# satoken/ractip

Measured on NVIDIA B200. Metric: shuffled pairs/sec, probability stage of --zscore=12 (McCaskill in/out x2 + unpaired windows x2 + two-strand McCaskill), higher is better.
Workload: dtype f64

## Files before the change

### ractip_b200/csrc/api.cu

```cuda
#include <cuda_runtime.h>

#include <algorithm>
#include <cstdio>
#include <cstdlib>
#include <string>
#include <utility>
#include <vector>

#include "dev_model.h"
#include "kernels.h"
#include "plan.h"
#include "ractip_prob.h"

using rp::Problem;

struct rp_ctx {
  int device = 0;
  int sm_count = 0;
  int ctas_per_sm = 0;
  int ctas_per_sm1 = 0;
  int up_ctas_per_sm = 0;
  size_t smem_optin = 0;
  rp::RouteSettings route;
  rp::DevModel* d_model = nullptr;
// ... 397 lines not shown
  CU(cudaEventRecord(ctx->ev[0], st));
  int launches = 0;
  if (p.n_band[0] && p.n_band[1]) CU(cudaEventRecord(ctx->ev_fork, st));
  for (int k = 0; k < 2; k++) {
    if (!p.n_band[k]) continue;
    rp::BatchDev db = d;
    db.order = b->d_order + (k ? p.n_band[0] : 0); db.nprob = p.n_band[k];
    db.counter = b->d_counter + 1 + k;
    db.ws = ctx->ws + p.ws_band[k]; db.slot_stride = p.band_slot[k]; db.nslots = p.band_grid[k];
    cudaStream_t ls = st;
    if (k == 1 && p.n_band[0]) {
      CU(cudaStreamWaitEvent(ctx->side_stream, ctx->ev_fork, 0));
      ls = ctx->side_stream;
    }
    if (p.dom_kind == k) CU(cudaEventRecord(ctx->ev_dom[0], ls));
    CU(rp::launch_band(db, p.band_grid[k], rp::BAND_THREADS[k], p.band_smem[k], ls));
    if (p.dom_kind == k) { CU(cudaEventRecord(ctx->ev_dom[1], ls)); ctx->dom_timed = true; }
    if (k == 0 && p.split_fetch) CU(cudaEventRecord(ctx->ev_main, st));
    if (ls != st) {
      CU(cudaEventRecord(ctx->ev_join, ls));
      CU(cudaStreamWaitEvent(st, ctx->ev_join, 0));
    }
    launches++;
  }
  if (p.up_mode == 1) {
    rp::BatchDev du = d;
    du.order = b->d_order + n_bandall + p.n_general; du.nprob = p.n_defer;
    du.counter = b->d_counter + 3;
    CU(rp::launch_unstru(du, p.up_grid, st));
    launches++;
  }
  if (p.n_mcc > 0) {
    if (p.dom_kind == 2) CU(cudaEventRecord(ctx->ev_dom[0], st));
    bool launched = false;
    for (int G = p.cluster; G && !launched; G = G == 16 ? 8 : 0) {
      const int ncl = std::max(1, std::min({p.n_mcc, p.grid, ctx->sm_count / G}));
      if (rp::launch_mcc_cluster(d, ncl, G, st) == cudaSuccess) launched = true;
      else cudaGetLastError();
    }
    if (!launched) CU(rp::launch_mcc(d, p.grid, p.mcc_minb, st));
    if (p.dom_kind == 2) { CU(cudaEventRecord(ctx->ev_dom[1], st)); ctx->dom_timed = true; }
    launches++;
  }
  if (p.n_duplex > 0) {
    CU(rp::launch_duplex(d, p.grid, st));
    launches++;
  }
  CU(cudaEventRecord(ctx->ev[1], st));
#ifdef RP_TUNE
  if (ctx->profile) {
    long long h[64];
    CU(cudaMemcpyAsync(h, ctx->d_prof, sizeof h, cudaMemcpyDeviceToHost, st));
    CU(cudaStreamSynchronize(st));
    static const char* names[32] = {"stage", "prologue", "prologue2", "inside_A", "inside_B", "generic_in", "generic_out", "outside_A", "outside_B", "write_bp", "un_hairpin", "un_gaps0", "un_gaps1", "un_domrows", "un_domcols", "un_mltab", "un_windows", "write_hp", "logz", "band_A", "band_B", "collect", "un_hairpin.cells(t0)", "un_hairpin.specials(t0)", "finish_in.loads(t0)", "finish_in.rest(t0)", "bandA_in.head(t0)", "bandA_in.main(t0)", "bandA_in.tail(t0)", "bandA_out.PR(t0)", "bandA_out.need(t0)", "bandA_out.ML(t0)"};
    long long tot = 0;
    for (int k = 0; k < 22; k++) tot += h[k];
    for (int k = 0; k < 32; k++)
      if (h[32 + k]) std::fprintf(stderr, "[rp_profile] %-11s %6.2f%%  calls %9lld  cycles/call %9.0f\n", names[k], 100.0 * h[k] / tot, h[32 + k], (double)h[k] / h[32 + k]);
  }
#endif
  ctx->timing.kernel_launches = launches;
  ctx->timing_pending = true;
  ctx->timed_copies = false;
  return RP_OK;
}

int rp_batch_sync(rp_batch* b) {
  if (!b) return RP_ERR_ARG;
  rp_ctx* ctx = b->ctx;
  CU(cudaStreamSynchronize(ctx->stream));
  return RP_OK;
}

int rp_batch_fetch_dense(rp_batch* b, float* out, size_t out_floats) {
  if (!b || !out) return RP_ERR_ARG;
  rp_ctx* ctx = b->ctx;
  const rp::BatchPlan& p = b->plan;
  if (out_floats < p.total_floats) return fail(ctx, RP_ERR_CAPACITY, "rp_batch_fetch_dense: buffer too small");
  CU(cudaSetDevice(ctx->device));
  CU(cudaEventRecord(ctx->ev[2], ctx->stream));
  if (p.total_floats && p.split_fetch) {
    const size_t pitch = p.pair_stride * sizeof(float);
    CU(cudaStreamWaitEvent(ctx->copy_stream, ctx->ev_main, 0));
    for (const auto& sc : p.sect_long)
      CU(cudaMemcpy2DAsync(out + sc.first, pitch, b->d_dense + sc.first, pitch, sc.second * sizeof(float), (size_t)b->n_pairs,
                           cudaMemcpyDeviceToHost, ctx->copy_stream));
    CU(cudaEventRecord(ctx->ev_copy, ctx->copy_stream));
    for (const auto& sc : p.sect_short)
      CU(cudaMemcpy2DAsync(out + sc.first, pitch, b->d_dense + sc.first, pitch, sc.second * sizeof(float), (size_t)b->n_pairs,
                           cudaMemcpyDeviceToHost, ctx->stream));
    CU(cudaStreamWaitEvent(ctx->stream, ctx->ev_copy, 0));
  } else if (p.total_floats) {
    CU(cudaMemcpyAsync(out, b->d_dense, p.total_floats * sizeof(float), cudaMemcpyDeviceToHost, ctx->stream));
  }
  CU(cudaEventRecord(ctx->ev[3], ctx->stream));
  CU(cudaStreamSynchronize(ctx->stream));
  ctx->timed_copies = true;
  return RP_OK;
}

}

namespace {
int sparse_prepare(rp_batch* b) {
  rp_ctx* ctx = b->ctx;
  const int np = b->n_pairs;
  if (b->d_spairs || np == 0) return RP_OK;
  std::vector<rp::SparsePair> sp(np);
  for (int p = 0; p < np; p++) {
// ... 175 lines not shown
```

### ractip_b200/csrc/mcc_core.h

```cpp
#ifndef RP_MCC_CORE_H
#define RP_MCC_CORE_H

#include <math.h>
#include <stdint.h>

#include "dev_model.h"

#ifdef __CUDACC__
#define RP_HD __host__ __device__ __forceinline__
#else
#define RP_HD inline
#endif

#ifdef RP_TUNE
#define RP_DBG(c) ((c).dbg)
#define RP_PROF(c) ((c).prof)
#else
#define RP_DBG(c) 0
#define RP_PROF(c) (static_cast<long long*>(nullptr))
#endif

namespace rp {

enum { KIND_LINEAR = 0, KIND_COFOLD = 1, KIND_DUPLEX = 2 };

struct Problem {
  int seq_off;
  int n;
  int cp;
  int kind;
  int pair;
  int which;
  int max_w;
  int n1, n2;
  long long out_bp;
  long long out_up;
  long long out_hp;
  float th_hy;
  int defer_up;
  long long ws_off;
};
constexpr int RP_JOB_UNPAIRED = 0x40000000;

enum {
  T_Q = 0, T_QQ, T_QM, T_QM1, T_QM2, T_QB, T_QBI, T_QB1N, T_QBAU,
  T_OUT, T_OUTI, T_OUT1N, T_OUTAU, T_MC, T_PR, T_PRML, T_PMLB, T_PL,
  T_DG, T_RR, T_LL, T_XX,
  T_QS, T_PRB, T_MLB,
  T_QMR, T_PRMLR,
  T_LIST,
  T_COUNT
};
enum {
  V_SCALE = 0, V_MLB, V_HPW, V_SP3, V_SP4, V_SP6, V_U0, V_U1,
  V_COUNT
};

constexpr int RP_MAX_N = 12000;
RP_HD size_t table_elems(int n) { return (size_t)n * (size_t)(n + 1) + 8; }
RP_HD size_t vector_elems(int n) { return (size_t)n + 8; }
RP_HD size_t slot_doubles(int n) { return T_COUNT * table_elems(n) + V_COUNT * vector_elems(n); }

struct Ctx {
  const DevModel* M;
  const uint8_t* S;
  int n, cp, ld, kind, max_w;
  double* ws;
  unsigned te, ve;
  double invZ;
  int dbg;
  long long* prof;
  RP_HD static constexpr unsigned ring_mask(int t) {
    return (t == T_PR || t == T_PL || t == T_PMLB) ? 1u : (t == T_QS || t == T_PRB || t == T_MLB) ? 15u : 0xffffffffu;
  }
  RP_HD unsigned off(int t, int d, int i) const { return (unsigned)t * te + ((unsigned)d & ring_mask(t)) * (unsigned)ld + (unsigned)i; }
  RP_HD double& tb(int t, int d, int i) const { return ws[off(t, d, i)]; }
  RP_HD double* ptr(int t, int d, int i) const { return ws + off(t, d, i); }
  RP_HD double* rptr(int t, int i, int j) const { return ws + ((unsigned)t * te + (unsigned)(i - 1) * (unsigned)ld + (unsigned)j); }
  RP_HD double& v(int vv, int k) const { return ws[(unsigned)T_COUNT * te + (unsigned)vv * ve + (unsigned)k]; }
  RP_HD int dstep() const { return ld; }
  RP_HD int pstep() const { return 1; }
  RP_HD int sraw(int i) const { return S[i]; }
};

RP_HD void bind_ctx(Ctx& c, const DevModel* M, const uint8_t* S, const Problem& p, double* ws) {
  c.M = M; c.S = S; c.n = p.n; c.cp = p.cp; c.ld = p.n + 1; c.kind = p.kind; c.max_w = p.max_w;
  c.ws = ws; c.te = (unsigned)table_elems(p.n); c.ve = (unsigned)vector_elems(p.n);
  c.invZ = 0;
  c.dbg = 0;
  c.prof = nullptr;
}
#define TB(c, t, d, i) ((c).tb(t, d, i))
#ifdef __CUDA_ARCH__
#define RP_ST_STREAM(ref, v) __stcs(&(ref), (v))
#else
#define RP_ST_STREAM(ref, v) ((ref) = (v))
#endif
#define VEC(c, vec_id, k) ((c).v(vec_id, k))

RP_HD uint16_t* listp(const Ctx& c) { return reinterpret_cast<uint16_t*>(c.ptr(T_LIST, 0, 0)); }
RP_HD uint16_t* posp(const Ctx& c) { return reinterpret_cast<uint16_t*>(c.ptr(T_LIST, 0, 0)) + c.te * 2; }

constexpr int BAND = TURN + 2;
constexpr int WIDE_MAX = 15;

constexpr int RP_SMEM_SEQ = 4096;
struct Shared {
  int T;
  double* part;
  double* grow;
  double* ghead_b;
  double* ghead_1;
  double* red;
  uint8_t* S;
  double* gtile;
  double* gpart;
};
constexpr int GS_ROW0 = 6, GS_NROWS = MAXLOOP - GS_ROW0 + 1;
RP_HD int gs_lt(int T) { return (T + MAXLOOP + 8 + 7) / 8 * 8; }
constexpr int GS_KINDS = 5;
RP_HD size_t gs_doubles(int T) { return (size_t)GS_KINDS * T + (size_t)GS_NROWS * gs_lt(T) + 8 * (size_t)T; }
RP_HD size_t part_doubles(int T, int W) {
  const size_t far = 2 * (size_t)W * T;
  return (W > BAND && gs_doubles(T) > far) ? gs_doubles(T) : far;
}
RP_HD size_t shared_bytes(int T, int W = BAND) {
  return sizeof(double) * (part_doubles(T, W) + (MAXLOOP + 1) * GROW_LD + 2 * GROW_LD + 128) + RP_SMEM_SEQ + 16;
}
RP_HD void carve_shared(Shared& sh, void* base, int T, int W = BAND) {
  sh.T = T;
  double* p = static_cast<double*>(base);
  sh.part = p; p += part_doubles(T, W);
// ... 1130 lines not shown
  }
}
template <int SIGN>
RP_HD void generic_items(const Ctx& c, const Shared& sh, int d, int i0, int C, int tid) {
  const int T = sh.T, LT = gs_lt(T), L8 = LT / 8;
  const GSplit gs = make_gsplit(C, T);
  const int warp = tid >> 5, lane = tid & 31;
  const int blk = warp / gs.wpb, bin = warp - blk * gs.wpb;
  if (blk >= gs.nb) return;
  const int g = blk * 32 + lane;
  const int smax = gs_smax(c.n, d, SIGN), nrows = smax - GS_ROW0 + 1;
  double tot[8];
#pragma unroll
  for (int r = 0; r < 8; r++) tot[r] = 0.;
  if (g < gs.NG) {
    for (int idx = bin; idx < nrows; idx += gs.wpb) {
      const int s = (idx & 1) ? GS_ROW0 + (idx >> 1) : smax - (idx >> 1);
      const double* row = sh.gtile + (size_t)(s - GS_ROW0) * LT + g;
#define RP_GX(cc) (((cc) & 7) * L8 + ((cc) >> 3))
      double win[8];
#pragma unroll
      for (int r = 0; r < 7; r++) win[r] = row[RP_GX(2 + r)];
      win[7] = 0.;
      const int nst = s - 3;
      int x = 0;
#pragma unroll 1
      for (; x + 8 <= nst; x += 8) {
#pragma unroll
        for (int u = 0; u < 8; u++) {
          win[(u + 7) & 7] = row[RP_GX(9 + u) + (x >> 3)];
          const double gv = sh.grow[(2 + x + u) * GROW_LD + (s - 2 - x - u)];
#pragma unroll
          for (int r = 0; r < 8; r++) tot[r] += gv * win[(u + r) & 7];
        }
      }
#pragma unroll
      for (int u = 0; u < 7; u++) {
        if (x + u < nst) {
          win[(u + 7) & 7] = row[RP_GX(9 + u) + (x >> 3)];
          const double gv = sh.grow[(2 + x + u) * GROW_LD + (s - 2 - x - u)];
#pragma unroll
          for (int r = 0; r < 8; r++) tot[r] += gv * win[(u + r) & 7];
        }
      }
#undef RP_GX
    }
  }
#pragma unroll
  for (int r = 0; r < 8; r++)
    if (8 * g + r < gs.cap) sh.gpart[(size_t)bin * gs.cap + 8 * g + r] = tot[r];
}

template <class C>
RP_HD void unstru_hairpin(C& c, int tid, int T) {
  const int n = c.n;
  const unsigned total = (unsigned)n * (unsigned)c.ld, ld = (unsigned)c.ld;
  for (unsigned x = tid; x < total; x += T) {
    const int d = (int)(x / ld), i = (int)(x - (unsigned)d * ld);
    if (i < 1 || i + d > n) continue;
    double v = 0.;
    if (d > TURN) {
      const double o = TB(c, T_OUT, d, i);
      if (o != 0.) v = o * hairpin(c, i, i + d, pair_type(base(c, i), base(c, i + d)));
    }
    TB(c, T_DG, d, i) = v;
  }
}
RP_HD int loop_class(int u1, int u2) {
  const int ul = u1 > u2 ? u1 : u2, us = u1 > u2 ? u2 : u1;
  if (us == 0) return ul >= 2 ? CLS_BULGE : CLS_SPECIAL;
  if (us == 1) return ul >= 3 ? CLS_1N : CLS_SPECIAL;
  return (us == 2 && (ul == 2 || ul == 3)) ? CLS_SPECIAL : CLS_GENERIC;
}

RP_HD int gap_special_slices(int n) { return n >= 48 ? 4 : 1; }
template <class C, class MT>
RP_HD void unstru_gap_specials(C& c, const MT& M, int tid, int T) {
  const int n = c.n;
  if (n < 7) return;
  const int nsl = gap_special_slices(n);
  const int items = (RP_DBG(c) & 4) ? 0 : 2 * 3 * nsl * n;
  for (int x = tid; x < items; x += T) {
    const int a = x % n + 1;
    int y = x / n;
    const int sl = y % nsl; y /= nsl;
    const int ug = y % 3 + 1, side = y / 3;
    const int b = a + ug + 1;
    double acc = 0.;
    if (b <= n) {
      if (side == 0) {
        const int p = a, k = b, u1 = ug, lmin = k + TURN + 1;
        const int sp1 = base(c, k - 1), si1 = base(c, p + 1);
        for (int u2 = 0; u2 <= 3; u2++) {
          if (loop_class(u1, u2) != CLS_SPECIAL) continue;
          const int lmax = n - 1 - u2, sidx = special_index(u1, u2);
          for (int l0 = lmin + sl; l0 <= lmax; l0 += 4 * nsl) {
            double qb[4], ou[4];
#pragma unroll
            for (int u = 0; u < 4; u++) {
              const int l = l0 + u * nsl;
              const bool on = l <= lmax;
              qb[u] = on ? TB(c, T_QB, l - k, k) : 0.;
              ou[u] = on ? TB(c, T_OUT, l + 1 + u2 - p, p) : 0.;
            }
            double w[4];
#pragma unroll
            for (int u = 0; u < 4; u++) {
              const int l = l0 + u * nsl <= lmax ? l0 + u * nsl : lmax, o = l + 1 + u2;
              w[u] = special_loop(M, sidx, pair_type(base(c, p), base(c, o)), rtype(pair_type(base(c, k), base(c, l))),
                                  si1, base(c, o - 1), sp1, base(c, l + 1));
            }
#pragma unroll
            for (int u = 0; u < 4; u++) acc += ou[u] * qb[u] * w[u];
          }
        }
      } else {
        const int l = a, o = b, u2 = ug;
        const int sq1 = base(c, l + 1), sj1 = base(c, o - 1);
        for (int u1 = 0; u1 <= 3; u1++) {
          if (loop_class(u1, u2) != CLS_SPECIAL) continue;
          const int pmax = l - TURN - 2 - u1, sidx = special_index(u1, u2);
          for (int p0 = 1 + sl; p0 <= pmax; p0 += 4 * nsl) {
            double qb[4], ou[4];
#pragma unroll
            for (int u = 0; u < 4; u++) {
              const int p = p0 + u * nsl;
              const bool on = p <= pmax;
              ou[u] = on ? TB(c, T_OUT, o - p, p) : 0.;
              qb[u] = on ? TB(c, T_QB, l - (p + 1 + u1), p + 1 + u1) : 0.;
            }
            double w[4];
#pragma unroll
            for (int u = 0; u < 4; u++) {
              const int p = p0 + u * nsl <= pmax ? p0 + u * nsl : pmax, k = p + 1 + u1;
              w[u] = special_loop(M, sidx, pair_type(base(c, p), base(c, o)), rtype(pair_type(base(c, k), base(c, l))),
                                  base(c, p + 1), sj1, base(c, k - 1), sq1);
            }
#pragma unroll
            for (int u = 0; u < 4; u++) acc += ou[u] * qb[u] * w[u];
          }
        }
      }
    }
    TB(c, T_RR, ((side * 3 + ug - 1) * nsl + sl), a) = acc;
  }
}

template <class C>
RP_HD void unstru_gaps(C& c, const double* gfull, int side, int tid, int T) {
  const int n = c.n, ds = c.dstep(), ps = c.pstep();
  const int items = (RP_DBG(c) & 4) ? 0 : n * (MAXLOOP + 1);
  const int tabO[3] = {T_OUTI, T_OUT1N, T_OUTAU};
  const int tabQ[3] = {T_QBI, T_QB1N, T_QBAU};
  for (int x = tid; x < items; x += T) {
    const int ug = x / n;
    const int a = x % n + 1;
    const int b = a + ug + 1;
    if (b > n || ug < 1) continue;
    double acc = 0.;
    if (side == 0) {
      const int p = a, k = b, u1 = ug;
      const int lmin = k + TURN + 1;
      for (int u2 = 0; u1 + u2 <= MAXLOOP;) {
        if (n - 1 - u2 < lmin) break;
        const int cls = loop_class(u1, u2);
        if (cls != CLS_SPECIAL) {
          int nu = 1;
          while (nu < 8 && u1 + u2 + nu <= MAXLOOP && loop_class(u1, u2 + nu) == cls && n - 1 - (u2 + nu) >= lmin) nu++;
          double av[8] = {0., 0., 0., 0., 0., 0., 0., 0.};
          const double* Q = c.ptr(tabQ[cls], lmin - k, k);
          const double* O = c.ptr(tabO[cls], lmin + 1 + u2 - p, p);
          const int cmain = n - 1 - (u2 + nu - 1) - lmin + 1;
          const int X = cmain + nu - 1;
          if (nu == 1) av[0] = dot_range(Q, ds, O, ds, 0, X, 0, 1);
          else multi_dot_slide(Q, ds, O, ds, X, 0, X - 1, av);
          for (int t = 0; t < nu; t++) acc += gfull[u1 * GROW_LD + u2 + t] * av[t];
          u2 += nu;
        } else {
          u2++;
        }
      }
    } else {
      const int l = a, o = b, u2 = ug;
      for (int u1 = 0; u1 + u2 <= MAXLOOP;) {
        if (l - TURN - 2 - u1 < 1) break;
        const int cls = loop_class(u1, u2);
        if (cls != CLS_SPECIAL) {
          int nu = 1;
          while (nu < 8 && u1 + nu + u2 <= MAXLOOP && loop_class(u1 + nu, u2) == cls && l - TURN - 2 - (u1 + nu) >= 1) nu++;
          double av[8] = {0., 0., 0., 0., 0., 0., 0., 0.};
          const double* O = c.ptr(tabO[cls], o - 1, 1);
          const double* Q = c.ptr(tabQ[cls], l - 2 - u1, 2 + u1);
          const int cmain = l - TURN - 2 - (u1 + nu - 1);
          if (cmain > 0) {
            const long st = ps - ds;
            const int X = cmain + nu - 1;
            if (nu == 1) {
              av[0] = dot_range(O + (long)(X - 1) * st, (int)-st, Q + (long)(X - 1) * st, (int)-st, 0, X, 0, 1);
            } else {
              double rv[8] = {0., 0., 0., 0., 0., 0., 0., 0.};
              multi_dot_slide(O + (long)(X - 1) * st, -st, Q + (long)(X + 6) * st, -st, X, 7, X + 6, rv);
#pragma unroll
              for (int t = 0; t < 8; t++) av[t] = rv[7 - t];
            }
          }
          for (int t = 0; t < nu; t++) acc += gfull[(u1 + t) * GROW_LD + u2] * av[t];
          u1 += nu;
        } else {
          u1++;
        }
      }
    }
    if (ug <= 3 && n >= 7) {
      const int nsl = gap_special_slices(n);
      for (int sl = 0; sl < nsl; sl++) acc += TB(c, T_RR, ((side * 3 + ug - 1) * nsl + sl), a);
    }
    TB(c, T_DG, b - a, a) += acc;
  }
}
template <class C>
RP_HD void unstru_dom_rows(C& c, int tid, int T) {
  const int n = c.n;
  for (int a = 1 + tid; a <= n; a += T) {
    double s = 0.;
    for (int b = n; b > a; b--) {
      s += TB(c, T_DG, b - a, a);
      TB(c, T_DG, b - a, a) = s;
    }
  }
}
template <class C>
RP_HD void unstru_dom_cols(C& c, int tid, int T) {
  const int n = c.n;
  for (int b = 2 + tid; b <= n; b += T) {
    double s = 0.;
    for (int a = 1; a < b; a++) {
      s += TB(c, T_DG, b - a, a);
      TB(c, T_DG, b - a, a) = s;
    }
  }
}
template <class C>
RP_HD void unstru_ml_tables(C& c, int tid, int T) {
  const int n = c.n;
  const double mlb1 = c.M->mlb1;
  for (int p0 = 1; p0 < n; p0 += T) {
    const int p = p0 + tid;
    double s = 0.;
#pragma unroll 8
    for (int d = n - p0; d >= 1; d--) {
      if (d > n - p) continue;
      const double mc = TB(c, T_MC, d, p);
      TB(c, T_LL, d, p) = s;
      s = s * mlb1 + mc;
    }
  }
  for (int o0 = 2; o0 <= n; o0 += T) {
    const int o = o0 + tid, top = (o0 + T - 1 < n ? o0 + T - 1 : n) - 1;
    double s = 0.;
#pragma unroll 8
    for (int d = top; d >= 1; d--) {
      if (o > n || d > o - 1) continue;
      const double mc = TB(c, T_MC, d, o - d);
      TB(c, T_RR, d, o - d) = s;
      s = mlb1 * (s + mc);
    }
  }
}
template <class C>
RP_HD void unstru_windows(C& c, float* up, int tid, int T) {
  const int n = c.n, w = c.max_w;
  for (int x = tid; x < n * w; x += T) {
    const int dd = x / n, i = x % n + 1, j = i + dd;
    double v = 0.;
    if (j <= n) {
      const double q5 = i > 1 ? TB(c, T_Q, i - 2, 1) : 1.0;
      const double q3 = j < n ? TB(c, T_Q, n - j - 1, j + 1) : 1.0;
      v = q5 * VEC(c, V_SCALE, dd + 1) * q3 * c.invZ;
      if (i > 1 && j < n) {
        v += TB(c, T_DG, j - i + 2, i - 1);
        double m1 = 0., m2 = 0., m3 = 0.;
        {
          const double* A = c.ptr(T_QM2, 2 * TURN + 3, j + 1);
          const double* B = c.ptr(T_RR, dd + 2 * TURN + 5, i);
          const int cnt = n - j - 2 - (2 * TURN + 3) + 1, ds = c.dstep();
#pragma unroll 4
          for (int t = 0; t < cnt; t++) m1 += A[(long)t * ds] * B[(long)t * ds];
        }
        {
          const int cnt = i - 3 - TURN, st = c.dstep() - c.pstep();
          const double* A2 = c.ptr(T_QM2, TURN + 1, i - 2 - TURN);
          const double* A1 = c.ptr(T_QM, TURN + 1, i - 2 - TURN);
          const double* BL = c.ptr(T_LL, dd + TURN + 3, i - 3 - TURN);
          const double* BR = c.ptr(T_XX, dd + TURN + 3, i - 3 - TURN);
#pragma unroll 4
          for (int t = 0; t < cnt; t++) {
            m2 += A2[(long)t * st] * BL[(long)t * st];
            m3 += A1[(long)t * st] * BR[(long)t * st];
          }
        }
        v += (m1 * VEC(c, V_MLB, dd) + (m2 + m3) * VEC(c, V_MLB, dd + 1)) * VEC(c, V_SCALE, 2);
      }
    }
    RP_ST_STREAM(up[(size_t)(i - 1) * w + dd], (float)v);
  }
}

template <class C>
RP_HD void write_bp(const C& c, float* bp, int tid, int T) {
  const int L = c.n;
  const size_t total = (size_t)(L + 1) * (L + 2) / 2;
  for (size_t x = tid; x < total; x += T) RP_ST_STREAM(bp[x], 0.f);
}
template <class C>
RP_HD void write_bp2(const C& c, float* bp, int tid, int T) {
  const int L = c.n;
  const unsigned total = (unsigned)L * (unsigned)c.ld, ld = (unsigned)c.ld;
  for (unsigned x = tid; x < total; x += T) {
// ... 28 lines not shown
```

### ractip_b200/csrc/mcc_driver.h

```cpp
#ifndef RP_MCC_DRIVER_H
#define RP_MCC_DRIVER_H

#include <type_traits>

#include "mcc_band.h"
#include "mcc_core.h"
#ifdef __CUDACC__
#include "mcc_band_shfl.cuh"
#include "mcc_wide_shfl.cuh"
#endif

namespace rp {

enum {
  PH_STAGE = 0, PH_PROLOGUE, PH_PROLOGUE2, PH_INSIDE_A, PH_INSIDE_B, PH_GENERIC_IN, PH_GENERIC_OUT, PH_OUTSIDE_A, PH_OUTSIDE_B,
  PH_WRITE_BP, PH_UN_HAIRPIN, PH_UN_GAPS0, PH_UN_GAPS1, PH_UN_DOMROWS, PH_UN_DOMCOLS, PH_UN_MLTAB, PH_UN_WINDOWS,
  PH_WRITE_HP, PH_LOGZ, PH_BAND_A, PH_BAND_B, PH_CFAC, PH_COUNT
};

template <class Exec, class = void>
struct CtasOf { static constexpr int value = 1; };
template <class Exec>
struct CtasOf<Exec, std::void_t<decltype(Exec::kCtas)>> { static constexpr int value = Exec::kCtas; };

RP_HD int deal_chunk(int total, int G, int cap) {
  int ch = (total + G - 1) / G;
  if (ch > cap) ch = cap;
  return ch < 1 ? 1 : ch;
}

template <class Exec, class F>
RP_HD void chunks(Exec& ex, int first, int end, int cap, F body) {
  constexpr int G = CtasOf<Exec>::value;
  const int ch = deal_chunk(end - first, G, cap);
  if constexpr (G == 1) {
    for (int i0 = first; i0 < end; i0 += ch) body(i0, end - i0 < ch ? end - i0 : ch);
  } else {
    for (int r = ex.rank_begin(); r < ex.rank_end(); r++)
      for (int i0 = first + r * ch; i0 < end; i0 += G * ch) body(i0, end - i0 < ch ? end - i0 : ch);
    ex.sync();
  }
}

template <class Exec, class F>
RP_HD void flat(Exec& ex, int id, F f) {
  constexpr int G = CtasOf<Exec>::value;
  const int T = ex.nthreads();
  if constexpr (G == 1) {
    ex.phase(id, [&](int tid) { f(tid, tid, T); });
  } else {
    for (int r = ex.rank_begin(); r < ex.rank_end(); r++) ex.phase(id, [&](int tid) { f(tid, r * T + tid, G * T); });
    ex.sync();
  }
}

template <class Exec, class F>
RP_HD void stage_sequence(Exec& ex, Ctx& c, uint8_t* S, F with) {
  const uint8_t* gS = c.S;
  const int n = c.n, T = ex.nthreads();
  ex.phase(PH_STAGE, [&](int tid) {
    for (int x = tid; x <= n + 1; x += T) S[x] = gS[x];
    with(tid);
  });
  c.S = S;
}

template <class Exec>
RP_HD void emit_logz(Exec& ex, Ctx& c, const Problem& p, double* logz) {
  if (!logz) return;
// ... 4 lines not shown
    if (tid == 0) logz[(size_t)p.pair * 3 + p.which] = log(TB(c, T_Q, c.n - 1, 1)) + c.n * log(c.M->pf_scale);
  });
}

template <int W, class Exec>
RP_HD void split_sums_inside(Exec& ex, Ctx& c, const Shared& sh, int d) {
  chunks(ex, 1, c.n - d + 1, wide_chunk<W>(sh.T), [&](int i0, int C) {
    ex.phase(PH_BAND_A, [&](int tid) {
#ifdef __CUDA_ARCH__
      if constexpr (W == BAND) inside_band_A_shfl<Exec::kBatch>(c, sh, d, i0, C, tid);
      else wide_inside_A_shfl<W, WIDE_NB>(c, sh, d, i0, C, tid);
#else
      if constexpr (W == BAND) inside_band_A(c, sh, d, i0, C, tid);
      else wide_inside_A<W>(c, sh, d, i0, C, tid);
#endif
    });
    ex.phase(PH_BAND_B, [&](int tid) {
#ifdef __CUDA_ARCH__
      if constexpr (W == BAND) inside_band_B_shfl(c, sh, d, i0, C, tid);
      else wide_inside_B_shfl<W>(c, sh, d, i0, C, tid);
#else
      if constexpr (W == BAND) inside_band_B(c, sh, d, i0, C, tid);
      else wide_inside_B<W>(c, sh, d, i0, C, tid);
#endif
    });
  });
}
template <int W, class Exec>
RP_HD void split_sums_outside(Exec& ex, Ctx& c, const Shared& sh, int d) {
  chunks(ex, 0, c.n - d + W - 1, wide_chunk<W>(sh.T), [&](int r0, int C) {
    ex.phase(PH_BAND_A, [&](int tid) {
#ifdef __CUDA_ARCH__
      if constexpr (W == BAND) outside_band_A_shfl<Exec::kBatch>(c, sh, d, r0, C, tid);
      else wide_outside_A_shfl<W, WIDE_NB>(c, sh, d, r0, C, tid);
#else
      if constexpr (W == BAND) outside_band_A(c, sh, d, r0, C, tid);
      else wide_outside_A<W>(c, sh, d, r0, C, tid);
#endif
    });
    ex.phase(PH_BAND_B, [&](int tid) {
#ifdef __CUDA_ARCH__
      if constexpr (W == BAND) outside_band_B_shfl(c, sh, d, r0, C, tid);
      else wide_outside_B_shfl<W>(c, sh, d, r0, C, tid);
#else
      if constexpr (W == BAND) outside_band_B(c, sh, d, r0, C, tid);
      else wide_outside_B<W>(c, sh, d, r0, C, tid);
#endif
    });
  });
}

template <class Exec, class MT>
RP_HD void emit_unpaired(Exec& ex, Ctx& c, const Problem& p, float* dense, const MT& SM, const double* gfull) {
  flat(ex, PH_UN_HAIRPIN, [&](int tid, int gt, int GT) {
#ifdef __CUDA_ARCH__
    long long* prof = RP_PROF(c);
    const long long t0 = (prof && tid == 0) ? clock64() : 0;
#endif
    unstru_hairpin(c, gt, GT);
#ifdef __CUDA_ARCH__
    const long long t1 = (prof && tid == 0) ? clock64() : 0;
#endif
    unstru_gap_specials(c, SM, gt, GT);
#ifdef __CUDA_ARCH__
    if (prof && tid == 0) {
      atomicAdd(reinterpret_cast<unsigned long long*>(prof + 22), (unsigned long long)(t1 - t0));
      atomicAdd(reinterpret_cast<unsigned long long*>(prof + 32 + 22), 1ull);
      atomicAdd(reinterpret_cast<unsigned long long*>(prof + 23), (unsigned long long)(clock64() - t1));
      atomicAdd(reinterpret_cast<unsigned long long*>(prof + 32 + 23), 1ull);
    }
#endif
  });
  flat(ex, PH_UN_GAPS0, [&](int, int gt, int GT) { unstru_gaps(c, gfull, 0, gt, GT); });
  flat(ex, PH_UN_GAPS1, [&](int, int gt, int GT) { unstru_gaps(c, gfull, 1, gt, GT); });
  flat(ex, PH_UN_DOMROWS, [&](int, int gt, int GT) { unstru_dom_rows(c, gt, GT); });
  flat(ex, PH_UN_DOMCOLS, [&](int, int gt, int GT) { unstru_dom_cols(c, gt, GT); });
  flat(ex, PH_UN_MLTAB, [&](int, int gt, int GT) { unstru_ml_tables(c, gt, GT); });
  if (p.out_up >= 0) flat(ex, PH_UN_WINDOWS, [&](int, int gt, int GT) { unstru_windows(c, dense + p.out_up, gt, GT); });
}

template <class Exec, class MT>
RP_HD void emit_outputs(Exec& ex, Ctx& c, const Problem& p, float* dense, const MT& SM, const double* gfull) {
  if (p.kind == KIND_LINEAR) {
    if (p.out_bp >= 0) {
      flat(ex, PH_WRITE_BP, [&](int, int gt, int GT) { write_bp(c, dense + p.out_bp, gt, GT); });
      flat(ex, PH_WRITE_BP, [&](int, int gt, int GT) { write_bp2(c, dense + p.out_bp, gt, GT); });
    }
    if (p.max_w > 0 && !p.defer_up) emit_unpaired(ex, c, p, dense, SM, gfull);
  } else if (p.kind == KIND_COFOLD) {
    if (p.out_hp >= 0)
      flat(ex, PH_WRITE_HP, [&](int, int gt, int GT) { write_hp(c, dense + p.out_hp, p.n1, p.n2, p.th_hy, gt, GT); });
  }
}

template <class Exec>
RP_HD void solve_mcc(Exec& ex, Ctx& c, const Problem& p, float* dense, double* logz, const Shared& sh) {
  const int T = sh.T;
  const int n = c.n;
  if (n + 2 <= RP_SMEM_SEQ) stage_sequence(ex, c, sh.S, [](int) {});
  ex.phase(PH_PROLOGUE, [&](int tid) {
    load_shared_model(*c.M, sh, tid);
    prologue_vectors(c, tid, T);
    prologue_lists(c, tid, T);
  });
  ex.phase(PH_PROLOGUE2, [&](int tid) { prologue2(c, tid, T); });

  for (int d = TURN + 1; d <= n - 1; d++) {
    if (d == band_start_inside(d)) split_sums_inside<BAND>(ex, c, sh, d);
    const int cells = n - d;
    const int chunk = cells < T ? cells : T;
    for (int i0 = 1; i0 <= cells; i0 += chunk) {
      const int C = cells - i0 + 1 < chunk ? cells - i0 + 1 : chunk;
      ex.phase(PH_INSIDE_A, [&](int tid) { inside_A(c, sh, d, i0, C, tid); });
      ex.phase(PH_INSIDE_B, [&](int tid) { inside_B(c, sh, d, i0, C, tid); });
    }
  }
  inside_end(c);
  emit_logz(ex, c, p, logz);

  for (int d = n - 1; d >= TURN + 1; d--) {
    if ((n - 1 - d) % BAND == 0) split_sums_outside<BAND>(ex, c, sh, d);
    const int lo = cross_lo(c, d), hi = cross_hi(c, d), cells = hi - lo + 1;
    const int chunk = cells < T ? cells : T;
    for (int i0 = lo; i0 <= hi; i0 += chunk) {
      const int C = hi - i0 + 1 < chunk ? hi - i0 + 1 : chunk;
      ex.phase(PH_OUTSIDE_A, [&](int tid) { outside_A(c, sh, d, i0, C, tid); });
      ex.phase(PH_OUTSIDE_B, [&](int tid) { outside_B(c, sh, d, i0, C, tid); });
    }
  }
  emit_outputs(ex, c, p, dense, *c.M, &c.M->gfull[0][0]);
// ... 148 lines not shown
```

Before: 27560.

## Fuse unpaired-probability phases into one work-item pass with scratch buffer

```diff
diff --git a/ractip_b200/csrc/api.cu b/ractip_b200/csrc/api.cu
--- a/ractip_b200/csrc/api.cu
+++ b/ractip_b200/csrc/api.cu
@@ -473,9 +473,9 @@
     long long h[64];
     CU(cudaMemcpyAsync(h, ctx->d_prof, sizeof h, cudaMemcpyDeviceToHost, st));
     CU(cudaStreamSynchronize(st));
-    static const char* names[32] = {"stage", "prologue", "prologue2", "inside_A", "inside_B", "generic_in", "generic_out", "outside_A", "outside_B", "write_bp", "un_hairpin", "un_gaps0", "un_gaps1", "un_domrows", "un_domcols", "un_mltab", "un_windows", "write_hp", "logz", "band_A", "band_B", "collect", "un_hairpin.cells(t0)", "un_hairpin.specials(t0)", "finish_in.loads(t0)", "finish_in.rest(t0)", "bandA_in.head(t0)", "bandA_in.main(t0)", "bandA_in.tail(t0)", "bandA_out.PR(t0)", "bandA_out.need(t0)", "bandA_out.ML(t0)"};
+    static const char* names[32] = {"stage", "prologue", "prologue2", "inside_A", "inside_B", "generic_in", "generic_out", "outside_A", "outside_B", "write_bp", "un_items", "un_domrows", "un_domcols", "un_windows", "write_hp", "logz", "band_A", "band_B", "collect", "", "", "", "", "", "finish_in.loads(t0)", "finish_in.rest(t0)", "bandA_in.head(t0)", "bandA_in.main(t0)", "bandA_in.tail(t0)", "bandA_out.PR(t0)", "bandA_out.need(t0)", "bandA_out.ML(t0)"};
     long long tot = 0;
-    for (int k = 0; k < 22; k++) tot += h[k];
+    for (int k = 0; k < 19; k++) tot += h[k];
     for (int k = 0; k < 32; k++)
       if (h[32 + k]) std::fprintf(stderr, "[rp_profile] %-11s %6.2f%%  calls %9lld  cycles/call %9.0f\n", names[k], 100.0 * h[k] / tot, h[32 + k], (double)h[k] / h[32 + k]);
   }
diff --git a/ractip_b200/csrc/mcc_core.h b/ractip_b200/csrc/mcc_core.h
--- a/ractip_b200/csrc/mcc_core.h
+++ b/ractip_b200/csrc/mcc_core.h
@@ -59,7 +59,9 @@
 constexpr int RP_MAX_N = 12000;
 RP_HD size_t table_elems(int n) { return (size_t)n * (size_t)(n + 1) + 8; }
 RP_HD size_t vector_elems(int n) { return (size_t)n + 8; }
-RP_HD size_t slot_doubles(int n) { return T_COUNT * table_elems(n) + V_COUNT * vector_elems(n); }
+constexpr int UP_SLICES_MAX = 4;
+RP_HD size_t up_scratch_elems(int n) { return (size_t)(2 * (MAXLOOP + 1) + 2 * 3 * UP_SLICES_MAX) * n + 8; }
+RP_HD size_t slot_doubles(int n) { return T_COUNT * table_elems(n) + V_COUNT * vector_elems(n) + up_scratch_elems(n); }
 
 struct Ctx {
   const DevModel* M;
@@ -78,6 +80,7 @@
   RP_HD double* ptr(int t, int d, int i) const { return ws + off(t, d, i); }
   RP_HD double* rptr(int t, int i, int j) const { return ws + ((unsigned)t * te + (unsigned)(i - 1) * (unsigned)ld + (unsigned)j); }
   RP_HD double& v(int vv, int k) const { return ws[(unsigned)T_COUNT * te + (unsigned)vv * ve + (unsigned)k]; }
+  RP_HD double* up_scratch() const { return ws + ((unsigned)T_COUNT * te + (unsigned)V_COUNT * ve); }
   RP_HD int dstep() const { return ld; }
   RP_HD int pstep() const { return 1; }
   RP_HD int sraw(int i) const { return S[i]; }
@@ -1314,19 +1317,17 @@
 }
 
 template <class C>
-RP_HD void unstru_hairpin(C& c, int tid, int T) {
+RP_HD void unstru_hairpin_cell(C& c, unsigned x) {
   const int n = c.n;
-  const unsigned total = (unsigned)n * (unsigned)c.ld, ld = (unsigned)c.ld;
-  for (unsigned x = tid; x < total; x += T) {
-    const int d = (int)(x / ld), i = (int)(x - (unsigned)d * ld);
-    if (i < 1 || i + d > n) continue;
-    double v = 0.;
-    if (d > TURN) {
-      const double o = TB(c, T_OUT, d, i);
-      if (o != 0.) v = o * hairpin(c, i, i + d, pair_type(base(c, i), base(c, i + d)));
-    }
-    TB(c, T_DG, d, i) = v;
-  }
+  const unsigned ld = (unsigned)c.ld;
+  const int d = (int)(x / ld), i = (int)(x - (unsigned)d * ld);
+  if (i < 1 || i + d > n) return;
+  double v = 0.;
+  if (d > TURN) {
+    const double o = TB(c, T_OUT, d, i);
+    if (o != 0.) v = o * hairpin(c, i, i + d, pair_type(base(c, i), base(c, i + d)));
+  }
+  TB(c, T_DG, d, i) = v;
 }
 RP_HD int loop_class(int u1, int u2) {
   const int ul = u1 > u2 ? u1 : u2, us = u1 > u2 ? u2 : u1;
@@ -1335,159 +1336,278 @@
   return (us == 2 && (ul == 2 || ul == 3)) ? CLS_SPECIAL : CLS_GENERIC;
 }
 
+RP_HD unsigned up_gap_idx(int n, int side, int ug, int a) {
+  return ((unsigned)side * (unsigned)n + (unsigned)(a - 1)) * (MAXLOOP + 1) + (unsigned)ug;
+}
+RP_HD unsigned up_special_idx(int n, int side, int ug, int nsl, int sl, int a) {
+  return 2u * (MAXLOOP + 1) * (unsigned)n + (unsigned)((side * 3 + ug - 1) * nsl + sl) * (unsigned)n + (unsigned)(a - 1);
+}
+
 RP_HD int gap_special_slices(int n) { return n >= 48 ? 4 : 1; }
 template <class C, class MT>
-RP_HD void unstru_gap_specials(C& c, const MT& M, int tid, int T) {
+RP_HD void unstru_gap_special(C& c, const MT& M, int x) {
   const int n = c.n;
-  if (n < 7) return;
   const int nsl = gap_special_slices(n);
-  const int items = (RP_DBG(c) & 4) ? 0 : 2 * 3 * nsl * n;
-  for (int x = tid; x < items; x += T) {
-    const int a = x % n + 1;
-    int y = x / n;
-    const int sl = y % nsl; y /= nsl;
-    const int ug = y % 3 + 1, side = y / 3;
-    const int b = a + ug + 1;
-    double acc = 0.;
-    if (b <= n) {
-      if (side == 0) {
-        const int p = a, k = b, u1 = ug, lmin = k + TURN + 1;
-        const int sp1 = base(c, k - 1), si1 = base(c, p + 1);
-        for (int u2 = 0; u2 <= 3; u2++) {
-          if (loop_class(u1, u2) != CLS_SPECIAL) continue;
-          const int lmax = n - 1 - u2, sidx = special_index(u1, u2);
-          for (int l0 = lmin + sl; l0 <= lmax; l0 += 4 * nsl) {
-            double qb[4], ou[4];
-#pragma unroll
-            for (int u = 0; u < 4; u++) {
-              const int l = l0 + u * nsl;
-              const bool on = l <= lmax;
-              qb[u] = on ? TB(c, T_QB, l - k, k) : 0.;
-              ou[u] = on ? TB(c, T_OUT, l + 1 + u2 - p, p) : 0.;
-            }
-            double w[4];
-#pragma unroll
-            for (int u = 0; u < 4; u++) {
-              const int l = l0 + u * nsl <= lmax ? l0 + u * nsl : lmax, o = l + 1 + u2;
-              w[u] = special_loop(M, sidx, pair_type(base(c, p), base(c, o)), rtype(pair_type(base(c, k), base(c, l))),
-                                  si1, base(c, o - 1), sp1, base(c, l + 1));
-            }
-#pragma unroll
-            for (int u = 0; u < 4; u++) acc += ou[u] * qb[u] * w[u];
+  const int a = x % n + 1;
+  int y = x / n;
+  const int sl = y % nsl; y /= nsl;
+  const int ug = y % 3 + 1, side = y / 3;
+  const int b = a + ug + 1;
+  double acc = 0.;
+  if (b <= n) {
+    if (side == 0) {
+      const int p = a, k = b, u1 = ug, lmin = k + TURN + 1;
+      const int sp1 = base(c, k - 1), si1 = base(c, p + 1);
+      for (int u2 = 0; u2 <= 3; u2++) {
+        if (loop_class(u1, u2) != CLS_SPECIAL) continue;
+        const int lmax = n - 1 - u2, sidx = special_index(u1, u2);
+        for (int l0 = lmin + sl; l0 <= lmax; l0 += 4 * nsl) {
+          double qb[4], ou[4];
+#pragma unroll
+          for (int u = 0; u < 4; u++) {
+            const int l = l0 + u * nsl;
+            const bool on = l <= lmax;
+            qb[u] = on ? TB(c, T_QB, l - k, k) : 0.;
+            ou[u] = on ? TB(c, T_OUT, l + 1 + u2 - p, p) : 0.;
+          }
+          double w[4];
+#pragma unroll
+          for (int u = 0; u < 4; u++) {
+            const int l = l0 + u * nsl <= lmax ? l0 + u * nsl : lmax, o = l + 1 + u2;
+            w[u] = special_loop(M, sidx, pair_type(base(c, p), base(c, o)), rtype(pair_type(base(c, k), base(c, l))),
+                                si1, base(c, o - 1), sp1, base(c, l + 1));
+          }
+#pragma unroll
+          for (int u = 0; u < 4; u++) acc += ou[u] * qb[u] * w[u];
+        }
+      }
+    } else {
+      const int l = a, o = b, u2 = ug;
+      const int sq1 = base(c, l + 1), sj1 = base(c, o - 1);
+      for (int u1 = 0; u1 <= 3; u1++) {
+        if (loop_class(u1, u2) != CLS_SPECIAL) continue;
+        const int pmax = l - TURN - 2 - u1, sidx = special_index(u1, u2);
+        for (int p0 = 1 + sl; p0 <= pmax; p0 += 4 * nsl) {
+          double qb[4], ou[4];
+#pragma unroll
+          for (int u = 0; u < 4; u++) {
+            const int p = p0 + u * nsl;
+            const bool on = p <= pmax;
+            ou[u] = on ? TB(c, T_OUT, o - p, p) : 0.;
+            qb[u] = on ? TB(c, T_QB, l - (p + 1 + u1), p + 1 + u1) : 0.;
+          }
+          double w[4];
+#pragma unroll
+          for (int u = 0; u < 4; u++) {
+            const int p = p0 + u * nsl <= pmax ? p0 + u * nsl : pmax, k = p + 1 + u1;
+            w[u] = special_loop(M, sidx, pair_type(base(c, p), base(c, o)), rtype(pair_type(base(c, k), base(c, l))),
+                                base(c, p + 1), sj1, base(c, k - 1), sq1);
+          }
+#pragma unroll
+          for (int u = 0; u < 4; u++) acc += ou[u] * qb[u] * w[u];
+        }
+      }
+    }
+  }
+  c.up_scratch()[up_special_idx(n, side, ug, nsl, sl, a)] = acc;
+}
+
+template <class C>
+RP_HD void unstru_gap_item(C& c, const double* gfull, int x) {
+  const int n = c.n, ds = c.dstep(), ps = c.pstep();
+  static_assert(MAXLOOP <= 32, "gap sizes per block of ranks");
+  const int side = (x >> 5) & 1, ug = ((x >> 6) & 31) + 1, r = (x >> 11 << 5) | (x & 31);
+  if (ug > MAXLOOP || r + ug > n - 2) return;
+  const int a = side ? n - 1 - r - ug : 1 + r;
+  const int b = a + ug + 1;
+  static_assert(T_OUT1N == T_OUTI + CLS_1N && T_OUTAU == T_OUTI + CLS_BULGE && T_QB1N == T_QBI + CLS_1N &&
+                T_QBAU == T_QBI + CLS_BULGE && CLS_GENERIC == 0, "class table order");
+  double acc = 0.;
+  if (side == 0) {
+    const int p = a, k = b, u1 = ug;
+    const int lmin = k + TURN + 1;
+    for (int u2 = 0; u1 + u2 <= MAXLOOP;) {
+      if (n - 1 - u2 < lmin) break;
+      const int cls = loop_class(u1, u2);
+      if (cls != CLS_SPECIAL) {
+        int nu = 1;
+        while (nu < 8 && u1 + u2 + nu <= MAXLOOP && loop_class(u1, u2 + nu) == cls && n - 1 - (u2 + nu) >= lmin) nu++;
+        double av[8] = {0., 0., 0., 0., 0., 0., 0., 0.};
+        const double* Q = c.ptr(T_QBI + cls, lmin - k, k);
+        const double* O = c.ptr(T_OUTI + cls, lmin + 1 + u2 - p, p);
+        const int cmain = n - 1 - (u2 + nu - 1) - lmin + 1;
+        const int X = cmain + nu - 1;
+        if (nu == 1) av[0] = dot_range(Q, ds, O, ds, 0, X, 0, 1);
+        else multi_dot_slide(Q, ds, O, ds, X, 0, X - 1, av);
+        for (int t = 0; t < nu; t++) acc += gfull[u1 * GROW_LD + u2 + t] * av[t];
+        u2 += nu;
+      } else {
+        u2++;
+      }
+    }
+    c.up_scratch()[up_gap_idx(n, 0, u1, p)] = acc;
+  } else {
+    const int l = a, o = b, u2 = ug;
+    for (int u1 = 0; u1 + u2 <= MAXLOOP;) {
+      if (l - TURN - 2 - u1 < 1) break;
+      const int cls = loop_class(u1, u2);
+      if (cls != CLS_SPECIAL) {
+        int nu = 1;
+        while (nu < 8 && u1 + nu + u2 <= MAXLOOP && loop_class(u1 + nu, u2) == cls && l - TURN - 2 - (u1 + nu) >= 1) nu++;
+        double av[8] = {0., 0., 0., 0., 0., 0., 0., 0.};
+        const double* O = c.ptr(T_OUTI + cls, o - 1, 1);
+        const double* Q = c.ptr(T_QBI + cls, l - 2 - u1, 2 + u1);
+        const int cmain = l - TURN - 2 - (u1 + nu - 1);
+        if (cmain > 0) {
+          const long st = ps - ds;
+          const int X = cmain + nu - 1;
+          if (nu == 1) {
+            av[0] = dot_range(O + (long)(X - 1) * st, (int)-st, Q + (long)(X - 1) * st, (int)-st, 0, X, 0, 1);
+          } else {
+            double rv[8] = {0., 0., 0., 0., 0., 0., 0., 0.};
+            multi_dot_slide(O + (long)(X - 1) * st, -st, Q + (long)(X + 6) * st, -st, X, 7, X + 6, rv);
+#pragma unroll
+            for (int t = 0; t < 8; t++) av[t] = rv[7 - t];
           }
         }
+        for (int t = 0; t < nu; t++) acc += gfull[(u1 + t) * GROW_LD + u2] * av[t];
+        u1 += nu;
       } else {
-        const int l = a, o = b, u2 = ug;
-        const int sq1 = base(c, l + 1), sj1 = base(c, o - 1);
-        for (int u1 = 0; u1 <= 3; u1++) {
-          if (loop_class(u1, u2) != CLS_SPECIAL) continue;
-          const int pmax = l - TURN - 2 - u1, sidx = special_index(u1, u2);
-          for (int p0 = 1 + sl; p0 <= pmax; p0 += 4 * nsl) {
-            double qb[4], ou[4];
-#pragma unroll
-            for (int u = 0; u < 4; u++) {
-              const int p = p0 + u * nsl;
-              const bool on = p <= pmax;
-              ou[u] = on ? TB(c, T_OUT, o - p, p) : 0.;
-              qb[u] = on ? TB(c, T_QB, l - (p + 1 + u1), p + 1 + u1) : 0.;
-            }
-            double w[4];
-#pragma unroll
-            for (int u = 0; u < 4; u++) {
-              const int p = p0 + u * nsl <= pmax ? p0 + u * nsl : pmax, k = p + 1 + u1;
-              w[u] = special_loop(M, sidx, pair_type(base(c, p), base(c, o)), rtype(pair_type(base(c, k), base(c, l))),
-                                  base(c, p + 1), sj1, base(c, k - 1), sq1);
-            }
-#pragma unroll
-            for (int u = 0; u < 4; u++) acc += ou[u] * qb[u] * w[u];
-          }
-        }
-      }
-    }
-    TB(c, T_RR, ((side * 3 + ug - 1) * nsl + sl), a) = acc;
-  }
-}
-
-template <class C>
-RP_HD void unstru_gaps(C& c, const double* gfull, int side, int tid, int T) {
-  const int n = c.n, ds = c.dstep(), ps = c.pstep();
-  const int items = (RP_DBG(c) & 4) ? 0 : n * (MAXLOOP + 1);
-  const int tabO[3] = {T_OUTI, T_OUT1N, T_OUTAU};
-  const int tabQ[3] = {T_QBI, T_QB1N, T_QBAU};
-  for (int x = tid; x < items; x += T) {
-    const int ug = x / n;
-    const int a = x % n + 1;
-    const int b = a + ug + 1;
-    if (b > n || ug < 1) continue;
-    double acc = 0.;
-    if (side == 0) {
-      const int p = a, k = b, u1 = ug;
-      const int lmin = k + TURN + 1;
-      for (int u2 = 0; u1 + u2 <= MAXLOOP;) {
-        if (n - 1 - u2 < lmin) break;
-        const int cls = loop_class(u1, u2);
-        if (cls != CLS_SPECIAL) {
-          int nu = 1;
-          while (nu < 8 && u1 + u2 + nu <= MAXLOOP && loop_class(u1, u2 + nu) == cls && n - 1 - (u2 + nu) >= lmin) nu++;
-          double av[8] = {0., 0., 0., 0., 0., 0., 0., 0.};
-          const double* Q = c.ptr(tabQ[cls], lmin - k, k);
-          const double* O = c.ptr(tabO[cls], lmin + 1 + u2 - p, p);
-          const int cmain = n - 1 - (u2 + nu - 1) - lmin + 1;
-          const int X = cmain + nu - 1;
-          if (nu == 1) av[0] = dot_range(Q, ds, O, ds, 0, X, 0, 1);
-          else multi_dot_slide(Q, ds, O, ds, X, 0, X - 1, av);
-          for (int t = 0; t < nu; t++) acc += gfull[u1 * GROW_LD + u2 + t] * av[t];
-          u2 += nu;
-        } else {
-          u2++;
-        }
-      }
-    } else {
-      const int l = a, o = b, u2 = ug;
-      for (int u1 = 0; u1 + u2 <= MAXLOOP;) {
-        if (l - TURN - 2 - u1 < 1) break;
-        const int cls = loop_class(u1, u2);
-        if (cls != CLS_SPECIAL) {
-          int nu = 1;
-          while (nu < 8 && u1 + nu + u2 <= MAXLOOP && loop_class(u1 + nu, u2) == cls && l - TURN - 2 - (u1 + nu) >= 1) nu++;
-          double av[8] = {0., 0., 0., 0., 0., 0., 0., 0.};
-          const double* O = c.ptr(tabO[cls], o - 1, 1);
-          const double* Q = c.ptr(tabQ[cls], l - 2 - u1, 2 + u1);
-          const int cmain = l - TURN - 2 - (u1 + nu - 1);
-          if (cmain > 0) {
-            const long st = ps - ds;
-            const int X = cmain + nu - 1;
-            if (nu == 1) {
-              av[0] = dot_range(O + (long)(X - 1) * st, (int)-st, Q + (long)(X - 1) * st, (int)-st, 0, X, 0, 1);
-            } else {
-              double rv[8] = {0., 0., 0., 0., 0., 0., 0., 0.};
-              multi_dot_slide(O + (long)(X - 1) * st, -st, Q + (long)(X + 6) * st, -st, X, 7, X + 6, rv);
-#pragma unroll
-              for (int t = 0; t < 8; t++) av[t] = rv[7 - t];
-            }
-          }
-          for (int t = 0; t < nu; t++) acc += gfull[(u1 + t) * GROW_LD + u2] * av[t];
-          u1 += nu;
-        } else {
-          u1++;
-        }
-      }
-    }
-    if (ug <= 3 && n >= 7) {
-      const int nsl = gap_special_slices(n);
-      for (int sl = 0; sl < nsl; sl++) acc += TB(c, T_RR, ((side * 3 + ug - 1) * nsl + sl), a);
-    }
-    TB(c, T_DG, b - a, a) += acc;
-  }
-}
+        u1++;
+      }
+    }
+    c.up_scratch()[up_gap_idx(n, 1, u2, l)] = acc;
+  }
+}
+
+constexpr int UP_NB = 8;
+template <class C>
+RP_HD void unstru_ml_row(C& c, int i) {
+  const int n = c.n, p = 1 + i, top = n - 1 - (i & ~31);
+  const double mlb1 = c.M->mlb1;
+  double s = 0.;
+  for (int d0 = top; d0 >= 1; d0 -= UP_NB) {
+    double mc[UP_NB];
+#pragma unroll
+    for (int u = 0; u < UP_NB; u++) mc[u] = d0 - u >= 1 && d0 - u <= n - p ? TB(c, T_MC, d0 - u, p) : 0.;
+#pragma unroll
+    for (int u = 0; u < UP_NB; u++) {
+      const int d = d0 - u;
+      if (d < 1 || d > n - p) continue;
+      TB(c, T_LL, d, p) = s;
+      s = s * mlb1 + mc[u];
+    }
+  }
+}
+template <class C>
+RP_HD void unstru_ml_col(C& c, int i) {
+  const int n = c.n, o = 2 + i, last = 2 + (i | 31), top = (last < n ? last : n) - 1;
+  const double mlb1 = c.M->mlb1;
+  double s = 0.;
+  for (int d0 = top; d0 >= 1; d0 -= UP_NB) {
+    double mc[UP_NB];
+#pragma unroll
+    for (int u = 0; u < UP_NB; u++) mc[u] = d0 - u >= 1 && d0 - u <= o - 1 ? TB(c, T_MC, d0 - u, o - (d0 - u)) : 0.;
+#pragma unroll
+    for (int u = 0; u < UP_NB; u++) {
+      const int d = d0 - u;
+      if (d < 1 || d > o - 1) continue;
+      TB(c, T_RR, d, o - d) = s;
+      s = mlb1 * (s + mc[u]);
+    }
+  }
+}
+
+template <class F>
+RP_HD void deal_snake(int first, int count, int gt, int GT, F body) {
+  const int end = first + count;
+  for (int k = first / GT; k * GT < end; k++) {
+    const int x = k * GT + ((k & 1) ? GT - 1 - gt : gt);
+    if (x >= first && x < end) body(x - first);
+  }
+}
+
+template <class C, class MT>
+RP_HD void unstru_items(C& c, const MT& M, const double* gfull, int gt, int GT) {
+  const int n = c.n;
+  const bool gaps = !(RP_DBG(c) & 4);
+  const int blocks = n > 2 ? (n - 2 + 31) / 32 : 0, blong = (blocks + 1) / 2;
+  const int nlong = gaps ? blong << 11 : 0, nshort = gaps ? (blocks - blong) << 11 : 0;
+  const int nscan = (n - 1 + 31) & ~31;
+  const int nspec = gaps && n >= 7 ? 2 * 3 * gap_special_slices(n) * n : 0;
+  const int xshort = nlong + 2 * nscan, xspec = xshort + nshort, xhp = xspec + nspec;
+  deal_snake(0, xspec, gt, GT, [&](int x) {
+    if (x < nlong || x >= xshort) unstru_gap_item(c, gfull, x < nlong ? x : x - 2 * nscan);
+  });
+  deal_snake(nlong, 2 * nscan, gt, GT, [&](int i) {
+    if (i < nscan) {
+      if (i < n - 1) unstru_ml_row(c, i);
+    } else if (i - nscan < n - 1) {
+      unstru_ml_col(c, i - nscan);
+    }
+  });
+  deal_snake(xspec, nspec, gt, GT, [&](int x) { unstru_gap_special(c, M, x); });
+  deal_snake(xhp, n * c.ld, gt, GT, [&](int x) { unstru_hairpin_cell(c, (unsigned)x); });
+}
+
 template <class C>
 RP_HD void unstru_dom_rows(C& c, int tid, int T) {
   const int n = c.n;
+  const bool gaps = !(RP_DBG(c) & 4), specials = gaps && n >= 7;
+  const int nsl = gap_special_slices(n);
+  const double* G = c.up_scratch();
   for (int a = 1 + tid; a <= n; a += T) {
+    double s0[3], s1[3];
+#pragma unroll
+    for (int g = 0; g < 3; g++) {
+      s0[g] = s1[g] = 0.;
+      if (gaps && a + g + 2 <= n) {
+        s0[g] = G[up_gap_idx(n, 0, g + 1, a)];
+        s1[g] = G[up_gap_idx(n, 1, g + 1, a)];
+        if (specials)
+          for (int sl = 0; sl < nsl; sl++) {
+            s0[g] += G[up_special_idx(n, 0, g + 1, nsl, sl, a)];
+            s1[g] += G[up_special_idx(n, 1, g + 1, nsl, sl, a)];
+          }
+      }
+    }
     double s = 0.;
-    for (int b = n; b > a; b--) {
-      s += TB(c, T_DG, b - a, a);
-      TB(c, T_DG, b - a, a) = s;
+    const int bnear = a + MAXLOOP + 1 < n ? a + MAXLOOP + 1 : n;
+    for (int b0 = n; b0 > bnear; b0 -= UP_NB) {
+      double v[UP_NB];
+#pragma unroll
+      for (int u = 0; u < UP_NB; u++) v[u] = b0 - u > bnear ? TB(c, T_DG, b0 - u - a, a) : 0.;
+#pragma unroll
+      for (int u = 0; u < UP_NB; u++) {
+        if (b0 - u <= bnear) continue;
+        s += v[u];
+        TB(c, T_DG, b0 - u - a, a) = s;
+      }
+    }
+    constexpr int NBN = UP_NB / 2;
+    for (int b0 = bnear; b0 > a; b0 -= NBN) {
+      double v[NBN], g0[NBN], g1[NBN];
+#pragma unroll
+      for (int u = 0; u < NBN; u++) {
+        const int b = b0 - u, ug = b - a - 1;
+        const bool gen = gaps && ug > 3;
+        v[u] = b > a ? TB(c, T_DG, b - a, a) : 0.;
+        g0[u] = gen ? G[up_gap_idx(n, 0, ug, a)] : 0.;
+        g1[u] = gen ? G[up_gap_idx(n, 1, ug, a)] : 0.;
+      }
+#pragma unroll
+      for (int u = 0; u < NBN; u++) {
+        const int b = b0 - u, ug = b - a - 1;
+        if (b <= a) continue;
+        double x = v[u];
+        if (gaps && ug >= 1) {
+          const double x0 = ug > 3 ? g0[u] : ug == 1 ? s0[0] : ug == 2 ? s0[1] : s0[2];
+          const double x1 = ug > 3 ? g1[u] : ug == 1 ? s1[0] : ug == 2 ? s1[1] : s1[2];
+          x = (x + x0) + x1;
+        }
+        s += x;
+        TB(c, T_DG, b - a, a) = s;
+      }
     }
   }
 }
@@ -1496,36 +1616,16 @@
   const int n = c.n;
   for (int b = 2 + tid; b <= n; b += T) {
     double s = 0.;
-    for (int a = 1; a < b; a++) {
-      s += TB(c, T_DG, b - a, a);
-      TB(c, T_DG, b - a, a) = s;
-    }
-  }
-}
-template <class C>
-RP_HD void unstru_ml_tables(C& c, int tid, int T) {
-  const int n = c.n;
-  const double mlb1 = c.M->mlb1;
-  for (int p0 = 1; p0 < n; p0 += T) {
-    const int p = p0 + tid;
-    double s = 0.;
-#pragma unroll 8
-    for (int d = n - p0; d >= 1; d--) {
-      if (d > n - p) continue;
-      const double mc = TB(c, T_MC, d, p);
-      TB(c, T_LL, d, p) = s;
-      s = s * mlb1 + mc;
-    }
-  }
-  for (int o0 = 2; o0 <= n; o0 += T) {
-    const int o = o0 + tid, top = (o0 + T - 1 < n ? o0 + T - 1 : n) - 1;
-    double s = 0.;
-#pragma unroll 8
-    for (int d = top; d >= 1; d--) {
-      if (o > n || d > o - 1) continue;
-      const double mc = TB(c, T_MC, d, o - d);
-      TB(c, T_RR, d, o - d) = s;
-      s = mlb1 * (s + mc);
+    for (int a0 = 1; a0 < b; a0 += UP_NB) {
+      double v[UP_NB];
+#pragma unroll
+      for (int u = 0; u < UP_NB; u++) v[u] = a0 + u < b ? TB(c, T_DG, b - a0 - u, a0 + u) : 0.;
+#pragma unroll
+      for (int u = 0; u < UP_NB; u++) {
+        if (a0 + u >= b) continue;
+        s += v[u];
+        TB(c, T_DG, b - a0 - u, a0 + u) = s;
+      }
     }
   }
 }
diff --git a/ractip_b200/csrc/mcc_driver.h b/ractip_b200/csrc/mcc_driver.h
--- a/ractip_b200/csrc/mcc_driver.h
+++ b/ractip_b200/csrc/mcc_driver.h
@@ -14,7 +14,7 @@
 
 enum {
   PH_STAGE = 0, PH_PROLOGUE, PH_PROLOGUE2, PH_INSIDE_A, PH_INSIDE_B, PH_GENERIC_IN, PH_GENERIC_OUT, PH_OUTSIDE_A, PH_OUTSIDE_B,
-  PH_WRITE_BP, PH_UN_HAIRPIN, PH_UN_GAPS0, PH_UN_GAPS1, PH_UN_DOMROWS, PH_UN_DOMCOLS, PH_UN_MLTAB, PH_UN_WINDOWS,
+  PH_WRITE_BP, PH_UN_ITEMS, PH_UN_DOMROWS, PH_UN_DOMCOLS, PH_UN_WINDOWS,
   PH_WRITE_HP, PH_LOGZ, PH_BAND_A, PH_BAND_B, PH_CFAC, PH_COUNT
 };
 
@@ -125,30 +125,9 @@
 
 template <class Exec, class MT>
 RP_HD void emit_unpaired(Exec& ex, Ctx& c, const Problem& p, float* dense, const MT& SM, const double* gfull) {
-  flat(ex, PH_UN_HAIRPIN, [&](int tid, int gt, int GT) {
-#ifdef __CUDA_ARCH__
-    long long* prof = RP_PROF(c);
-    const long long t0 = (prof && tid == 0) ? clock64() : 0;
-#endif
-    unstru_hairpin(c, gt, GT);
-#ifdef __CUDA_ARCH__
-    const long long t1 = (prof && tid == 0) ? clock64() : 0;
-#endif
-    unstru_gap_specials(c, SM, gt, GT);
-#ifdef __CUDA_ARCH__
-    if (prof && tid == 0) {
-      atomicAdd(reinterpret_cast<unsigned long long*>(prof + 22), (unsigned long long)(t1 - t0));
-      atomicAdd(reinterpret_cast<unsigned long long*>(prof + 32 + 22), 1ull);
-      atomicAdd(reinterpret_cast<unsigned long long*>(prof + 23), (unsigned long long)(clock64() - t1));
-      atomicAdd(reinterpret_cast<unsigned long long*>(prof + 32 + 23), 1ull);
-    }
-#endif
-  });
-  flat(ex, PH_UN_GAPS0, [&](int, int gt, int GT) { unstru_gaps(c, gfull, 0, gt, GT); });
-  flat(ex, PH_UN_GAPS1, [&](int, int gt, int GT) { unstru_gaps(c, gfull, 1, gt, GT); });
+  flat(ex, PH_UN_ITEMS, [&](int, int gt, int GT) { unstru_items(c, SM, gfull, gt, GT); });
   flat(ex, PH_UN_DOMROWS, [&](int, int gt, int GT) { unstru_dom_rows(c, gt, GT); });
   flat(ex, PH_UN_DOMCOLS, [&](int, int gt, int GT) { unstru_dom_cols(c, gt, GT); });
-  flat(ex, PH_UN_MLTAB, [&](int, int gt, int GT) { unstru_ml_tables(c, gt, GT); });
   if (p.out_up >= 0) flat(ex, PH_UN_WINDOWS, [&](int, int gt, int GT) { unstru_windows(c, dense + p.out_up, gt, GT); });
 }
 
```

After: 28660, median of 6. 1.04x the previous value.
